# ilur98/DLMC-QUANT

Hardware: AMD Instinct MI355X
Metric: ResNet-50 W8A8 fake-quant fwd images/sec (higher is better)
Workload: dtype i8; 1 GPU; resnet50 W8A8 per-channel fake-quant forward (FSPTQ forms: W minmax_channel s8, A minmax_tensor u8), BN folded first as in FSPTQuant.py:67, fused int8 MFMA conv/linear, frozen execution plan (epilogue-fused ReLU / shortcut / next-layer codes; block end + next 1x1 as one launch; weight codes quantised once at plan build), 2 HIP streams per GPU, 224x224 relu(N(0,1)) pixels, batch 512 per GPU, scales; global_batch=512, parallelism=dp1 (batch-sharded replicas)

## Files before the change

dlmc-quant_amd/csrc/conv_pw_i8.hip:

```cpp
#include "conv_i8_common.h"

namespace dlmcq {

struct PwArgs {
  const int8_t* x;
  const int8_t* w;
  const float* s_w;
  const int32_t* wsum;
  const float* bias;
  const float* s_in;
  const float* zp_in;
  int M, K, shift, nslice;
  int nblk;
  unsigned long long* trace;
};

constexpr int PW_WPS(int c, int bn) { return c >= 1024 ? 1 : (c >= 512 ? 3 : 4); }

template <int C, int BN, int NTP, bool ASYM, int NW, int LAB = 0, bool R6 = false>
__global__ __launch_bounds__(NW * 64, PW_WPS(C, BN)) void conv_pw_i8_kernel(PwArgs a, ConvEpi ep) {
  constexpr int S = C / 64;
  constexpr int NA = C / 32;
  constexpr int NT = BN / 32;
  constexpr int WB = C * BN;
  constexpr int PIECES = S * (BN / 16);
  constexpr int NPAR = ASYM ? 4 : 3;
  constexpr int NP = NT / NTP;
  constexpr int JP = NTP > 1 ? 1 : 0;
  static_assert(NT % NTP == 0 && JP < NTP && NTP >= 1, "the request sits inside the last pass's epilogue");
  extern __shared__ __attribute__((aligned(1024))) int8_t pw_lds[];
  int8_t* const wl = pw_lds;
  int8_t* const par = pw_lds + WB;
  constexpr int SROW = BN + 16;
  constexpr int LPR = BN / 16, RPI = 64 / LPR;
  constexpr int NST = (32 + RPI - 1) / RPI;
  int8_t* const stg = pw_lds + WB + 4 * BN * 4 + (threadIdx.x >> 6) * (32 * SROW);
  const int srow = (int)((threadIdx.x & 63) / LPR), sseg = (int)(threadIdx.x & 63) - srow * LPR;

  const int tid = threadIdx.x, wave = tid >> 6, lane = tid & 63, l31 = lane & 31, hsel = lane >> 5;
  const uint32_t b = blockIdx.x;
  const int slice = (int)((b >> 3) % (uint32_t)a.nslice);
  const int group = (int)((b >> 3) / (uint32_t)a.nslice) * 8 + (int)(b & 7u);
  const int ngroups = (int)(gridDim.x / (uint32_t)a.nslice);
  const int n0 = slice * BN;

  unsigned long long* tr = nullptr;
  if (LAB == 1 && a.trace && blockIdx.x == gridDim.x / 2 && tid == 0) tr = a.trace;
  int nstamp = 3;
  auto stamp = [&]() {
    if (LAB == 1 && tr && nstamp < 256) tr[nstamp++] = __builtin_readcyclecounter();
  };
  if (LAB == 1 && tr) tr[0] = __builtin_amdgcn_s_memrealtime();
  stamp();
  unsigned long long* wgt = nullptr;
  if (LAB == 1 && a.trace && tid == 0) {
    wgt = a.trace + 256 + 4 * (size_t)blockIdx.x;
    wgt[0] = __builtin_amdgcn_s_memrealtime();
    wgt[2] = __builtin_amdgcn_s_getreg(4 | (31 << 11));
    wgt[3] = __builtin_amdgcn_s_getreg(20 | (31 << 11));
  }
  {
    const void* arrs[4] = {a.s_w, a.wsum, a.bias, ASYM ? ep.w_off : nullptr};
#pragma unroll
    for (int r = 0; r < NPAR; ++r) {
      if (!arrs[r]) {
        for (int c = tid; c < BN; c += NW * 64) reinterpret_cast<float*>(par)[r * BN + c] = 0.0f;
        continue;
      }
      for (int c = wave; c < BN / 64; c += NW)
        __builtin_amdgcn_global_load_lds((gptr_t)(static_cast<const int32_t*>(arrs[r]) + n0 + c * 64 + lane), (lptr_t)(par + (r * BN + c * 64) * 4), 4, 0, 0);
    }
    const int lrow = lane >> 2, pslot = lane & 3;
    for (int pc = wave; pc < PIECES; pc += NW) {
      const int s = pc / (BN / 16), r16 = pc - s * (BN / 16);
      const int row = r16 * 16 + lrow;
      const int d = row & 31;
      const int k = n0 + (row & ~31) + 16 * ((d >> 2) & 1) + 4 * (d >> 3) + (d & 3);
      const int seg = pslot ^ ((row >> 2) & 3);
      __builtin_amdgcn_global_load_lds((gptr_t)(a.w + (int64_t)k * C + s * 64 + seg * 16), (lptr_t)(wl + s * (BN * 64) + r16 * 1024), 16, 0, 0);
    }
  }
  const float zpf = a.zp_in ? a.zp_in[0] : 0.0f;
  const int zpi = (int)__builtin_rintf(zpf);
  const float sin = a.s_in[0];
  const uint32_t xorw = a.shift ? 0x80808080u : 0u;
  const EpiQuant eq(ep, ep.relu != 0);
  const v4i r_x = make_rsrc(a.x, (uint32_t)((int64_t)a.M * C));
  const v4i r_c = make_rsrc(ep.codes, (uint32_t)((int64_t)a.M * a.K));

  i32x4 areg[NA];
  auto request = [&](int blk) {
    const int row = blk * 32 + l31;
    const int vo = (blk < a.nblk && row < a.M) ? row * C + hsel * 16 : BUF_BIG;
    if constexpr (LAB == 2) {
#pragma unroll
      for (int f = 0; f < NA; ++f) areg[f] = i32x4{vo, 1, 2, 3};
      return;
    }
    static_for<NA>([&](auto f) { bload16i<decltype(f)::value * 32>(areg[decltype(f)::value], vo, r_x); });
  };
  const int stride = ngroups * NW;
  int blk = group * NW + wave;
  request(blk);
  asm volatile("s_waitcnt vmcnt(0)" ::: "memory");
  __syncthreads();
  if (tid < BN) {
    float* pf = reinterpret_cast<float*>(par) + tid;
    int* pi = reinterpret_cast<int*>(par) + BN + tid;
    *pf = sin * *pf;
    *pi = (a.shift - zpi) * *pi;
    if constexpr (ASYM) pf[3 * BN] = sin * pf[3 * BN];
  }
  __syncthreads();

  stamp();
  for (; blk < a.nblk; blk += stride) {
    stamp();
    if constexpr (LAB == 2 || LAB == 7 || LAB == 8) asm volatile("s_waitcnt vmcnt(0)" ::: "memory");
    else asm volatile("s_waitcnt vmcnt(%0)" ::"n"(NST) : "memory");
    stamp();
#pragma unroll
    for (int f = 0; f < NA; ++f) {
      asm volatile("" : "+v"(areg[f]));
      areg[f] = i32x4{(int)(areg[f].x ^ xorw), (int)(areg[f].y ^ xorw), (int)(areg[f].z ^ xorw), (int)(areg[f].w ^ xorw)};
    }
    f32x2 s0f2 = f32x2{0.0f, 0.0f};
    static_for<NP>([&](auto p_c) {
      constexpr int p = decltype(p_c)::value;
      i32x16 acc[NTP];
#pragma unroll
      for (int j = 0; j < NTP; ++j) {
        const i32x4* cop = reinterpret_cast<const i32x4*>(par + (BN + (p * NTP + j) * 32 + hsel * 16) * 4);
#pragma unroll
        for (int q = 0; q < 4; ++q) {
          const i32x4 c4 = cop[q];
          acc[j][4 * q] = c4.x;
          acc[j][4 * q + 1] = c4.y;
          acc[j][4 * q + 2] = c4.z;
          acc[j][4 * q + 3] = c4.w;
        }
      }
      int s0 = 0;
      static_for<NA>([&](auto f_c) {
        constexpr int f = decltype(f_c)::value;
        constexpr int s = f >> 1, ks = f & 1;
        const i32x4 af = areg[f];
        if constexpr (ASYM && p == 0) {
          s0 = __builtin_amdgcn_sdot4(af.x, 0x01010101, s0, false);
          s0 = __builtin_amdgcn_sdot4(af.y, 0x01010101, s0, false);
          s0 = __builtin_amdgcn_sdot4(af.z, 0x01010101, s0, false);
          s0 = __builtin_amdgcn_sdot4(af.w, 0x01010101, s0, false);
        }
        const int sg = ks * 2 + hsel;
#pragma unroll
        for (int j = 0; j < NTP; ++j) {
          const int brow = (p * NTP + j) * 32 + l31;
          const i32x4 bf = *reinterpret_cast<const i32x4*>(wl + s * (BN * 64) + brow * 64 + ((sg ^ ((brow >> 2) & 3)) << 4));
          if constexpr (LAB == 4) asm volatile("" ::"v"(af), "v"(bf));
          else acc[j] = __builtin_amdgcn_mfma_i32_32x32x32_i8(bf, af, acc[j], 0, 0, 0);
        }
      });
      if constexpr (LAB == 1) {
        asm volatile("s_nop 0" ::"v"(acc[0][0]), "v"(acc[NTP - 1][15]));
        stamp();
      }
      if constexpr (ASYM && p == 0) {
        s0 += __shfl_xor(s0, 32, 64);
        s0 += (a.shift - zpi) * C;
        s0f2 = f32x2{(float)s0, (float)s0};
      }
#pragma unroll
      for (int jj = 0; jj < NTP; ++jj) {
        if (p == NP - 1 && jj == JP) request(blk + stride);
        const int j = p * NTP + jj;
        const int cb = j * 32 + hsel * 16;
        if constexpr (LAB == 6 || LAB == 7) {
          uint32_t wl4[4];
#pragma unroll
          for (int q = 0; q < 4; ++q)
            wl4[q] = (uint32_t)(acc[jj][4 * q] & 0xff) | ((uint32_t)(acc[jj][4 * q + 1] & 0xff) << 8) | ((uint32_t)(acc[jj][4 * q + 2] & 0xff) << 16) |
                     ((uint32_t)acc[jj][4 * q + 3] << 24);
          if constexpr (LAB == 6) *reinterpret_cast<i32x4*>(stg + l31 * SROW + cb) = i32x4{(int)wl4[0], (int)wl4[1], (int)wl4[2], (int)wl4[3]};
          else asm volatile("" ::"v"(wl4[0]), "v"(wl4[1]), "v"(wl4[2]), "v"(wl4[3]));
          continue;
        }
        f32x4 y[4];
#pragma unroll
        for (int q = 0; q < 4; ++q) {
          const f32x4 mu = *reinterpret_cast<const f32x4*>(par + (cb + 4 * q) * 4);
          const f32x4 bs = *reinterpret_cast<const f32x4*>(par + (2 * BN + cb + 4 * q) * 4);
          f32x2 ya = pk_fma(f32x2{(float)acc[jj][4 * q], (float)acc[jj][4 * q + 1]}, f32x2{mu.x, mu.y}, f32x2{bs.x, bs.y});
          f32x2 yb = pk_fma(f32x2{(float)acc[jj][4 * q + 2], (float)acc[jj][4 * q + 3]}, f32x2{mu.z, mu.w}, f32x2{bs.z, bs.w});
          if constexpr (ASYM) {
            const f32x4 wo = *reinterpret_cast<const f32x4*>(par + (3 * BN + cb + 4 * q) * 4);
            ya = ya + s0f2 * f32x2{wo.x, wo.y};
            yb = yb + s0f2 * f32x2{wo.z, wo.w};
          }
          y[q] = f32x4{ya.x, ya.y, yb.x, yb.y};
          if constexpr (R6) y[q] = cap6_nan4(y[q]);
        }
        uint32_t wq[4];
        eq.code4n_plain(y, wq);
        *reinterpret_cast<i32x4*>(stg + l31 * SROW + cb) = i32x4{(int)wq[0], (int)wq[1], (int)wq[2], (int)wq[3]};
      }
      stamp();
    });
    if constexpr (LAB != 7) {
      const int r0 = blk * 32 + srow;
      const int vbase = r0 * a.K + n0 + sseg * 16;
      const int8_t* const sbase = stg + srow * SROW + sseg * 16;
#pragma unroll
      for (int it = 0; it < NST; ++it) {
        const bool ok = srow < RPI && it * RPI + srow < 32 && r0 + it * RPI < a.M;
        const bool whole = (it + 1) * RPI <= 32;
        const i32x4 c16 = *reinterpret_cast<const i32x4*>(whole || it * RPI + srow < 32 ? sbase + it * RPI * SROW : stg + 31 * SROW + sseg * 16);
        if constexpr (LAB == 8) asm volatile("" ::"v"(c16));
        else if constexpr (LAB == 9) bstore16i_nt(c16, ok ? vbase + it * RPI * a.K : BUF_BIG, r_c);
        else bstore16i(c16, ok ? vbase + it * RPI * a.K : BUF_BIG, r_c);
      }
    }
    stamp();
  }
  if (LAB == 1 && tr) {
    asm volatile("s_waitcnt vmcnt(0)" ::: "memory");
    stamp();
    tr[1] = __builtin_amdgcn_s_memrealtime();
    tr[2] = (unsigned long long)nstamp;
  }
  if (LAB == 1 && wgt) {
    asm volatile("s_waitcnt vmcnt(0)" ::: "memory");
    wgt[1] = __builtin_amdgcn_s_memrealtime();
  }
  asm volatile("s_waitcnt vmcnt(0)" ::: "memory");
}

#define DLMCQ_PW_PAIRS(X) X(64, 64) X(64, 128) X(64, 192) X(128, 128) X(128, 192) X(192, 128) X(192, 192) X(512, 128) X(1024, 128)
constexpr int pw_slice(int64_t K) { return K == 192 ? 192 : (K == 64 ? 64 : (K % 128 == 0 ? 128 : 0)); }
constexpr bool pw_built(int64_t C, int bn) {
#define DLMCQ_PW_HAS(CC, BB) if (C == CC && bn == BB) return true;
  DLMCQ_PW_PAIRS(DLMCQ_PW_HAS)
#undef DLMCQ_PW_HAS
  return false;
}

bool conv_pw_applies(int64_t N, int64_t H, int64_t W, int64_t C, int64_t K, int64_t R, int64_t S, int32_t stride, int32_t pad,
                     int32_t dilation, const ConvEpi& ep, const float* out, bool dual) {
  if (R != 1 || S != 1 || stride != 1 || pad != 0 || dilation != 1 || dual || out || ep.residual || !ep.codes) return false;
  if (!epi_plain(ep)) return false;
  if (K > 1024 || !pw_built(C, pw_slice(K))) return false;
  if (!aligned16(ep.codes)) return false;
  const int64_t M = N * H * W;
  if (M < 4096) return false;
  if (M * C >= (int64_t)BUF_BIG || M * K >= (int64_t)BUF_BIG) return false;
  return true;
}

template <int C, int BN, bool ASYM, int LAB = 0, bool R6 = false>
static int pw_go(const PwArgs& a0, const ConvEpi& ep, hipStream_t st) {
  constexpr int WPS = PW_WPS(C, BN);
  constexpr int LDS1 = C * BN + 4 * BN * 4, STG = 4 * 32 * (BN + 16);
  constexpr bool BIGWG = C >= 1024 || (LDS1 + STG) * WPS > 158 * 1024;
  constexpr int NW = C >= 1024 ? 6 : (BIGWG ? 4 * WPS : 4);
  constexpr int LDS = LDS1 + NW * (STG / 4);
  static_assert(LDS <= 160 * 1024, "LDS");
  PwArgs a = a0;
  a.nslice = a.K / BN;
  static int cus = 0;
  if (!cus) {
    int dev = 0;
    hipDeviceProp_t prop;
    cus = (hipGetDevice(&dev) == hipSuccess && hipGetDeviceProperties(&prop, dev) == hipSuccess && prop.multiProcessorCount > 0)
              ? prop.multiProcessorCount : 256;
  }
  const int wgs = cus * (BIGWG ? 1 : WPS);
  int ngroups = (wgs / a.nslice) & ~7;
  if (ngroups < 8) ngroups = 8;
  const int maxg = ((a.nblk + NW - 1) / NW + 7) & ~7;
  if (ngroups > maxg) ngroups = maxg;
  constexpr int NTP = BN == 192 ? 3 : (C >= 512 ? 1 : 2);
  auto kern = conv_pw_i8_kernel<C, BN, NTP, ASYM, NW, LAB, R6>;
  static bool attr_set = false;
  if (!attr_set) {
    const hipError_t e = hipFuncSetAttribute(reinterpret_cast<const void*>(kern), hipFuncAttributeMaxDynamicSharedMemorySize, LDS);
    if (e != hipSuccess) return (int)e;
    attr_set = true;
  }
  hipLaunchKernelGGL(kern, dim3((uint32_t)(ngroups * a.nslice)), dim3(NW * 64), LDS, st, a, ep);
  return launch_status();
}

int conv_pw_launch(const int8_t* x, const int8_t* w, const float* bias, const int32_t* wsum, const float* in_scale,
                   const float* in_zero_point, const float* w_scale, int64_t N, int64_t H, int64_t W, int64_t C, int64_t K, int shift,
                   const ConvEpi& ep, hipStream_t st, int lab, void* lab_trace) {
  PwArgs a{};
  a.trace = static_cast<unsigned long long*>(lab_trace);
  a.x = x; a.w = w; a.s_w = w_scale; a.wsum = wsum; a.bias = bias; a.s_in = in_scale; a.zp_in = in_zero_point;
  a.M = (int)(N * H * W); a.K = (int)K; a.shift = shift;
  a.nblk = (a.M + 31) / 32;
  const bool asym = ep.w_off != nullptr;
  const int bn = pw_slice(K);
#ifdef DLMCQ_LAB
#define DLMCQ_PWL(CC, BB, L) \
  if (C == CC && bn == BB && lab == L && asym) return pw_go<CC, BB, true, L>(a, ep, st)
#define DLMCQ_PWLS(CC, BB) DLMCQ_PWL(CC, BB, 1); DLMCQ_PWL(CC, BB, 2); DLMCQ_PWL(CC, BB, 4); DLMCQ_PWL(CC, BB, 6); DLMCQ_PWL(CC, BB, 7); DLMCQ_PWL(CC, BB, 8); DLMCQ_PWL(CC, BB, 9)
  DLMCQ_PWLS(128, 128);
  DLMCQ_PWLS(192, 192);
  DLMCQ_PWLS(192, 128);
  DLMCQ_PWLS(512, 128);
#undef DLMCQ_PWLS
#undef DLMCQ_PWL
#endif
  if (lab) return DLMCQ_EINVAL;
  const bool r6 = ep.relu == DLMCQ_ACT_RELU6;
#define DLMCQ_PW(CC, BB)                                                                                       \
  if (C == CC && bn == BB)                                                                                     \
    return r6 ? (asym ? pw_go<CC, BB, true, 0, true>(a, ep, st) : pw_go<CC, BB, false, 0, true>(a, ep, st))     \
              : (asym ? pw_go<CC, BB, true>(a, ep, st) : pw_go<CC, BB, false>(a, ep, st));
  DLMCQ_PW_PAIRS(DLMCQ_PW)
#undef DLMCQ_PW
  return DLMCQ_EINVAL;
}

}
```

Measured before the change: 94170 images/s.

## Split pointwise conv K-loop into double-buffered halves for wide-C layers

Adds a KH template parameter that splits the activation fragments of the pointwise int8 kernel into KH parts, alternating between two register sets. The next part's loads are issued before the current part's MFMAs, so global loads overlap compute. This targets C=1024 and C=2048 inputs in ResNet-50, which now use a 64-wide output slice and a 2- or 4-way split, and C=2048 is newly routed to this kernel. The cost is more register pressure and different occupancy (two waves per SIMD). The epilogue is moved into a lambda and the CU count is now read through a shared helper.

```diff
diff --git a/dlmc-quant_amd/csrc/conv_pw_i8.hip b/dlmc-quant_amd/csrc/conv_pw_i8.hip
--- a/dlmc-quant_amd/csrc/conv_pw_i8.hip
+++ b/dlmc-quant_amd/csrc/conv_pw_i8.hip
@@ -15,12 +15,13 @@
   unsigned long long* trace;
 };
 
-constexpr int PW_WPS(int c, int bn) { return c >= 1024 ? 1 : (c >= 512 ? 3 : 4); }
-
-template <int C, int BN, int NTP, bool ASYM, int NW, int LAB = 0, bool R6 = false>
-__global__ __launch_bounds__(NW * 64, PW_WPS(C, BN)) void conv_pw_i8_kernel(PwArgs a, ConvEpi ep) {
+constexpr int PW_WPS(int c, int bn, int kh = 1) { return kh > 1 ? 2 : (c >= 1024 ? 1 : (c >= 512 ? 3 : 4)); }
+
+template <int C, int BN, int NTP, bool ASYM, int NW, int LAB = 0, bool R6 = false, int KH = 1>
+__global__ __launch_bounds__(NW * 64, PW_WPS(C, BN, KH)) void conv_pw_i8_kernel(PwArgs a, ConvEpi ep) {
   constexpr int S = C / 64;
   constexpr int NA = C / 32;
+  constexpr int NAH = NA / KH;
   constexpr int NT = BN / 32;
   constexpr int WB = C * BN;
   constexpr int PIECES = S * (BN / 16);
@@ -28,6 +29,7 @@
   constexpr int NP = NT / NTP;
   constexpr int JP = NTP > 1 ? 1 : 0;
   static_assert(NT % NTP == 0 && JP < NTP && NTP >= 1, "the request sits inside the last pass's epilogue");
+  static_assert(KH == 1 || (KH % 2 == 0 && NA % KH == 0 && NTP == NT && LAB == 0), "parts alternate between two fragment sets; one pass");
   extern __shared__ __attribute__((aligned(1024))) int8_t pw_lds[];
   int8_t* const wl = pw_lds;
   int8_t* const par = pw_lds + WB;
@@ -88,20 +90,22 @@
   const v4i r_x = make_rsrc(a.x, (uint32_t)((int64_t)a.M * C));
   const v4i r_c = make_rsrc(ep.codes, (uint32_t)((int64_t)a.M * a.K));
 
-  i32x4 areg[NA];
-  auto request = [&](int blk) {
+  i32x4 areg[KH > 1 ? 2 : 1][NAH];
+  auto request = [&](int blk, auto h_c, auto set_c) {
+    constexpr int h = decltype(h_c)::value, set = decltype(set_c)::value;
     const int row = blk * 32 + l31;
     const int vo = (blk < a.nblk && row < a.M) ? row * C + hsel * 16 : BUF_BIG;
     if constexpr (LAB == 2) {
 #pragma unroll
-      for (int f = 0; f < NA; ++f) areg[f] = i32x4{vo, 1, 2, 3};
+      for (int f = 0; f < NAH; ++f) areg[set][f] = i32x4{vo, 1, 2, 3};
       return;
     }
-    static_for<NA>([&](auto f) { bload16i<decltype(f)::value * 32>(areg[decltype(f)::value], vo, r_x); });
+    static_for<NAH>([&](auto f) { bload16i<(h * NAH + decltype(f)::value) * 32>(areg[set][decltype(f)::value], vo, r_x); });
   };
+  constexpr std::integral_constant<int, 0> i0{};
   const int stride = ngroups * NW;
   int blk = group * NW + wave;
-  request(blk);
+  request(blk, i0, i0);
   asm volatile("s_waitcnt vmcnt(0)" ::: "memory");
   __syncthreads();
   if (tid < BN) {
@@ -113,17 +117,53 @@
   }
   __syncthreads();
 
+  auto finish = [&](const i32x16& accj, const int j, const f32x2 s0f2) {
+    const int cb = j * 32 + hsel * 16;
+    if constexpr (LAB == 6 || LAB == 7) {
+      uint32_t wl4[4];
+#pragma unroll
+      for (int q = 0; q < 4; ++q)
+        wl4[q] = (uint32_t)(accj[4 * q] & 0xff) | ((uint32_t)(accj[4 * q + 1] & 0xff) << 8) | ((uint32_t)(accj[4 * q + 2] & 0xff) << 16) |
+                 ((uint32_t)accj[4 * q + 3] << 24);
+      if constexpr (LAB == 6) *reinterpret_cast<i32x4*>(stg + l31 * SROW + cb) = i32x4{(int)wl4[0], (int)wl4[1], (int)wl4[2], (int)wl4[3]};
+      else asm volatile("" ::"v"(wl4[0]), "v"(wl4[1]), "v"(wl4[2]), "v"(wl4[3]));
+      return;
+    }
+    f32x4 y[4];
+#pragma unroll
+    for (int q = 0; q < 4; ++q) {
+      const f32x4 mu = *reinterpret_cast<const f32x4*>(par + (cb + 4 * q) * 4);
+      const f32x4 bs = *reinterpret_cast<const f32x4*>(par + (2 * BN + cb + 4 * q) * 4);
+      f32x2 ya = pk_fma(f32x2{(float)accj[4 * q], (float)accj[4 * q + 1]}, f32x2{mu.x, mu.y}, f32x2{bs.x, bs.y});
+      f32x2 yb = pk_fma(f32x2{(float)accj[4 * q + 2], (float)accj[4 * q + 3]}, f32x2{mu.z, mu.w}, f32x2{bs.z, bs.w});
+      if constexpr (ASYM) {
+        const f32x4 wo = *reinterpret_cast<const f32x4*>(par + (3 * BN + cb + 4 * q) * 4);
+        ya = ya + s0f2 * f32x2{wo.x, wo.y};
+        yb = yb + s0f2 * f32x2{wo.z, wo.w};
+      }
+      y[q] = f32x4{ya.x, ya.y, yb.x, yb.y};
+      if constexpr (R6) y[q] = cap6_nan4(y[q]);
+    }
+    uint32_t wq[4];
+    eq.code4n_plain(y, wq);
+    *reinterpret_cast<i32x4*>(stg + l31 * SROW + cb) = i32x4{(int)wq[0], (int)wq[1], (int)wq[2], (int)wq[3]};
+  };
+  auto landed = [&](auto set_c, auto cnt_c) {
+    constexpr int set = decltype(set_c)::value;
+    if constexpr (LAB == 2 || LAB == 7 || LAB == 8) asm volatile("s_waitcnt vmcnt(0)" ::: "memory");
+    else asm volatile("s_waitcnt vmcnt(%0)" ::"n"(decltype(cnt_c)::value) : "memory");
+    stamp();
+#pragma unroll
+    for (int f = 0; f < NAH; ++f) {
+      asm volatile("" : "+v"(areg[set][f]));
+      areg[set][f] = i32x4{(int)(areg[set][f].x ^ xorw), (int)(areg[set][f].y ^ xorw), (int)(areg[set][f].z ^ xorw),
+                           (int)(areg[set][f].w ^ xorw)};
+    }
+  };
   stamp();
   for (; blk < a.nblk; blk += stride) {
     stamp();
-    if constexpr (LAB == 2 || LAB == 7 || LAB == 8) asm volatile("s_waitcnt vmcnt(0)" ::: "memory");
-    else asm volatile("s_waitcnt vmcnt(%0)" ::"n"(NST) : "memory");
-    stamp();
-#pragma unroll
-    for (int f = 0; f < NA; ++f) {
-      asm volatile("" : "+v"(areg[f]));
-      areg[f] = i32x4{(int)(areg[f].x ^ xorw), (int)(areg[f].y ^ xorw), (int)(areg[f].z ^ xorw), (int)(areg[f].w ^ xorw)};
-    }
+    if constexpr (KH == 1) landed(i0, std::integral_constant<int, NST>{});
     f32x2 s0f2 = f32x2{0.0f, 0.0f};
     static_for<NP>([&](auto p_c) {
       constexpr int p = decltype(p_c)::value;
@@ -141,24 +181,32 @@
         }
       }
       int s0 = 0;
-      static_for<NA>([&](auto f_c) {
-        constexpr int f = decltype(f_c)::value;
-        constexpr int s = f >> 1, ks = f & 1;
-        const i32x4 af = areg[f];
-        if constexpr (ASYM && p == 0) {
-          s0 = __builtin_amdgcn_sdot4(af.x, 0x01010101, s0, false);
-          s0 = __builtin_amdgcn_sdot4(af.y, 0x01010101, s0, false);
-          s0 = __builtin_amdgcn_sdot4(af.z, 0x01010101, s0, false);
-          s0 = __builtin_amdgcn_sdot4(af.w, 0x01010101, s0, false);
+      static_for<KH>([&](auto h_c) {
+        constexpr int h = decltype(h_c)::value, set = h & 1;
+        if constexpr (KH > 1) {
+          if constexpr (h + 1 < KH) request(blk, std::integral_constant<int, h + 1>{}, std::integral_constant<int, (h + 1) & 1>{});
+          else request(blk + stride, i0, i0);
+          landed(std::integral_constant<int, set>{}, std::integral_constant<int, (h == 0 ? NST : 0) + NAH>{});
         }
-        const int sg = ks * 2 + hsel;
-#pragma unroll
-        for (int j = 0; j < NTP; ++j) {
-          const int brow = (p * NTP + j) * 32 + l31;
-          const i32x4 bf = *reinterpret_cast<const i32x4*>(wl + s * (BN * 64) + brow * 64 + ((sg ^ ((brow >> 2) & 3)) << 4));
-          if constexpr (LAB == 4) asm volatile("" ::"v"(af), "v"(bf));
-          else acc[j] = __builtin_amdgcn_mfma_i32_32x32x32_i8(bf, af, acc[j], 0, 0, 0);
-        }
+        static_for<NAH>([&](auto f_c) {
+          constexpr int f = h * NAH + decltype(f_c)::value;
+          constexpr int s = f >> 1, ks = f & 1;
+          const i32x4 af = areg[set][decltype(f_c)::value];
+          if constexpr (ASYM && p == 0) {
+            s0 = __builtin_amdgcn_sdot4(af.x, 0x01010101, s0, false);
+            s0 = __builtin_amdgcn_sdot4(af.y, 0x01010101, s0, false);
+            s0 = __builtin_amdgcn_sdot4(af.z, 0x01010101, s0, false);
+            s0 = __builtin_amdgcn_sdot4(af.w, 0x01010101, s0, false);
+          }
+          const int sg = ks * 2 + hsel;
+#pragma unroll
+          for (int j = 0; j < NTP; ++j) {
+            const int brow = (p * NTP + j) * 32 + l31;
+            const i32x4 bf = *reinterpret_cast<const i32x4*>(wl + s * (BN * 64) + brow * 64 + ((sg ^ ((brow >> 2) & 3)) << 4));
+            if constexpr (LAB == 4) asm volatile("" ::"v"(af), "v"(bf));
+            else acc[j] = __builtin_amdgcn_mfma_i32_32x32x32_i8(bf, af, acc[j], 0, 0, 0);
+          }
+        });
       });
       if constexpr (LAB == 1) {
         asm volatile("s_nop 0" ::"v"(acc[0][0]), "v"(acc[NTP - 1][15]));
@@ -171,37 +219,8 @@
       }
 #pragma unroll
       for (int jj = 0; jj < NTP; ++jj) {
-        if (p == NP - 1 && jj == JP) request(blk + stride);
-        const int j = p * NTP + jj;
-        const int cb = j * 32 + hsel * 16;
-        if constexpr (LAB == 6 || LAB == 7) {
-          uint32_t wl4[4];
-#pragma unroll
-          for (int q = 0; q < 4; ++q)
-            wl4[q] = (uint32_t)(acc[jj][4 * q] & 0xff) | ((uint32_t)(acc[jj][4 * q + 1] & 0xff) << 8) | ((uint32_t)(acc[jj][4 * q + 2] & 0xff) << 16) |
-                     ((uint32_t)acc[jj][4 * q + 3] << 24);
-          if constexpr (LAB == 6) *reinterpret_cast<i32x4*>(stg + l31 * SROW + cb) = i32x4{(int)wl4[0], (int)wl4[1], (int)wl4[2], (int)wl4[3]};
-          else asm volatile("" ::"v"(wl4[0]), "v"(wl4[1]), "v"(wl4[2]), "v"(wl4[3]));
-          continue;
-        }
-        f32x4 y[4];
-#pragma unroll
-        for (int q = 0; q < 4; ++q) {
-          const f32x4 mu = *reinterpret_cast<const f32x4*>(par + (cb + 4 * q) * 4);
-          const f32x4 bs = *reinterpret_cast<const f32x4*>(par + (2 * BN + cb + 4 * q) * 4);
-          f32x2 ya = pk_fma(f32x2{(float)acc[jj][4 * q], (float)acc[jj][4 * q + 1]}, f32x2{mu.x, mu.y}, f32x2{bs.x, bs.y});
-          f32x2 yb = pk_fma(f32x2{(float)acc[jj][4 * q + 2], (float)acc[jj][4 * q + 3]}, f32x2{mu.z, mu.w}, f32x2{bs.z, bs.w});
-          if constexpr (ASYM) {
-            const f32x4 wo = *reinterpret_cast<const f32x4*>(par + (3 * BN + cb + 4 * q) * 4);
-            ya = ya + s0f2 * f32x2{wo.x, wo.y};
-            yb = yb + s0f2 * f32x2{wo.z, wo.w};
-          }
-          y[q] = f32x4{ya.x, ya.y, yb.x, yb.y};
-          if constexpr (R6) y[q] = cap6_nan4(y[q]);
-        }
-        uint32_t wq[4];
-        eq.code4n_plain(y, wq);
-        *reinterpret_cast<i32x4*>(stg + l31 * SROW + cb) = i32x4{(int)wq[0], (int)wq[1], (int)wq[2], (int)wq[3]};
+        if (KH == 1 && p == NP - 1 && jj == JP) request(blk + stride, i0, i0);
+        finish(acc[jj], p * NTP + jj, s0f2);
       }
       stamp();
     });
@@ -234,10 +253,16 @@
   asm volatile("s_waitcnt vmcnt(0)" ::: "memory");
 }
 
-#define DLMCQ_PW_PAIRS(X) X(64, 64) X(64, 128) X(64, 192) X(128, 128) X(128, 192) X(192, 128) X(192, 192) X(512, 128) X(1024, 128)
-constexpr int pw_slice(int64_t K) { return K == 192 ? 192 : (K == 64 ? 64 : (K % 128 == 0 ? 128 : 0)); }
-constexpr bool pw_built(int64_t C, int bn) {
-#define DLMCQ_PW_HAS(CC, BB) if (C == CC && bn == BB) return true;
+#define DLMCQ_PW_PAIRS(X)                                                                                                            \
+  X(64, 64, 1, true) X(64, 128, 1, true) X(64, 192, 1, true) X(128, 128, 1, true) X(128, 192, 1, true) X(192, 128, 1, true)          \
+  X(192, 192, 1, true) X(512, 128, 1, true) X(1024, 128, 1, true) X(1024, 64, 2, true) X(2048, 64, 4, false)
+constexpr int pw_slice(int64_t C, int64_t K) {
+  if ((C == 1024 || C == 2048) && K % 128 == 0 && K <= 512) return 64;
+  if (C == 2048) return 0;
+  return K == 192 ? 192 : (K == 64 ? (C < 1024 ? 64 : 0) : (K % 128 == 0 ? 128 : 0));
+}
+constexpr bool pw_built(int64_t C, int bn, bool asym) {
+#define DLMCQ_PW_HAS(CC, BB, HH, AS) if (C == CC && bn == BB) return AS || !asym;
   DLMCQ_PW_PAIRS(DLMCQ_PW_HAS)
 #undef DLMCQ_PW_HAS
   return false;
@@ -247,7 +272,7 @@
                      int32_t dilation, const ConvEpi& ep, const float* out, bool dual) {
   if (R != 1 || S != 1 || stride != 1 || pad != 0 || dilation != 1 || dual || out || ep.residual || !ep.codes) return false;
   if (!epi_plain(ep)) return false;
-  if (K > 1024 || !pw_built(C, pw_slice(K))) return false;
+  if (K > 1024 || !pw_built(C, pw_slice(C, K), ep.w_off != nullptr)) return false;
   if (!aligned16(ep.codes)) return false;
   const int64_t M = N * H * W;
   if (M < 4096) return false;
@@ -255,30 +280,23 @@
   return true;
 }
 
-template <int C, int BN, bool ASYM, int LAB = 0, bool R6 = false>
+template <int C, int BN, bool ASYM, int LAB = 0, bool R6 = false, int KH = 1>
 static int pw_go(const PwArgs& a0, const ConvEpi& ep, hipStream_t st) {
-  constexpr int WPS = PW_WPS(C, BN);
+  constexpr int WPS = PW_WPS(C, BN, KH);
   constexpr int LDS1 = C * BN + 4 * BN * 4, STG = 4 * 32 * (BN + 16);
   constexpr bool BIGWG = C >= 1024 || (LDS1 + STG) * WPS > 158 * 1024;
-  constexpr int NW = C >= 1024 ? 6 : (BIGWG ? 4 * WPS : 4);
+  constexpr int NW = KH > 1 ? 4 * WPS : (C >= 1024 ? 6 : (BIGWG ? 4 * WPS : 4));
   constexpr int LDS = LDS1 + NW * (STG / 4);
   static_assert(LDS <= 160 * 1024, "LDS");
   PwArgs a = a0;
   a.nslice = a.K / BN;
-  static int cus = 0;
-  if (!cus) {
-    int dev = 0;
-    hipDeviceProp_t prop;
-    cus = (hipGetDevice(&dev) == hipSuccess && hipGetDeviceProperties(&prop, dev) == hipSuccess && prop.multiProcessorCount > 0)
-              ? prop.multiProcessorCount : 256;
-  }
-  const int wgs = cus * (BIGWG ? 1 : WPS);
+  const int wgs = device_cus() * (BIGWG ? 1 : WPS);
   int ngroups = (wgs / a.nslice) & ~7;
   if (ngroups < 8) ngroups = 8;
   const int maxg = ((a.nblk + NW - 1) / NW + 7) & ~7;
   if (ngroups > maxg) ngroups = maxg;
-  constexpr int NTP = BN == 192 ? 3 : (C >= 512 ? 1 : 2);
-  auto kern = conv_pw_i8_kernel<C, BN, NTP, ASYM, NW, LAB, R6>;
+  constexpr int NTP = KH > 1 ? BN / 32 : (BN == 192 ? 3 : (C >= 512 ? 1 : 2));
+  auto kern = conv_pw_i8_kernel<C, BN, NTP, ASYM, NW, LAB, R6, KH>;
   static bool attr_set = false;
   if (!attr_set) {
     const hipError_t e = hipFuncSetAttribute(reinterpret_cast<const void*>(kern), hipFuncAttributeMaxDynamicSharedMemorySize, LDS);
@@ -287,6 +305,16 @@
   }
   hipLaunchKernelGGL(kern, dim3((uint32_t)(ngroups * a.nslice)), dim3(NW * 64), LDS, st, a, ep);
   return launch_status();
+}
+
+template <int C, int BN, int KH, bool AS>
+static int pw_pick(const PwArgs& a, const ConvEpi& ep, hipStream_t st) {
+  const bool r6 = ep.relu == DLMCQ_ACT_RELU6;
+  if (ep.w_off != nullptr) {
+    if constexpr (AS) return r6 ? pw_go<C, BN, true, 0, true, KH>(a, ep, st) : pw_go<C, BN, true, 0, false, KH>(a, ep, st);
+    else return DLMCQ_EINVAL;
+  }
+  return r6 ? pw_go<C, BN, false, 0, true, KH>(a, ep, st) : pw_go<C, BN, false, 0, false, KH>(a, ep, st);
 }
 
 int conv_pw_launch(const int8_t* x, const int8_t* w, const float* bias, const int32_t* wsum, const float* in_scale,
@@ -297,9 +325,9 @@
   a.x = x; a.w = w; a.s_w = w_scale; a.wsum = wsum; a.bias = bias; a.s_in = in_scale; a.zp_in = in_zero_point;
   a.M = (int)(N * H * W); a.K = (int)K; a.shift = shift;
   a.nblk = (a.M + 31) / 32;
+  const int bn = pw_slice(C, K);
+#ifdef DLMCQ_LAB
   const bool asym = ep.w_off != nullptr;
-  const int bn = pw_slice(K);
-#ifdef DLMCQ_LAB
 #define DLMCQ_PWL(CC, BB, L) \
   if (C == CC && bn == BB && lab == L && asym) return pw_go<CC, BB, true, L>(a, ep, st)
 #define DLMCQ_PWLS(CC, BB) DLMCQ_PWL(CC, BB, 1); DLMCQ_PWL(CC, BB, 2); DLMCQ_PWL(CC, BB, 4); DLMCQ_PWL(CC, BB, 6); DLMCQ_PWL(CC, BB, 7); DLMCQ_PWL(CC, BB, 8); DLMCQ_PWL(CC, BB, 9)
@@ -311,11 +339,8 @@
 #undef DLMCQ_PWL
 #endif
   if (lab) return DLMCQ_EINVAL;
-  const bool r6 = ep.relu == DLMCQ_ACT_RELU6;
-#define DLMCQ_PW(CC, BB)                                                                                       \
-  if (C == CC && bn == BB)                                                                                     \
-    return r6 ? (asym ? pw_go<CC, BB, true, 0, true>(a, ep, st) : pw_go<CC, BB, false, 0, true>(a, ep, st))     \
-              : (asym ? pw_go<CC, BB, true>(a, ep, st) : pw_go<CC, BB, false>(a, ep, st));
+#define DLMCQ_PW(CC, BB, HH, AS) \
+  if (C == CC && bn == BB) return pw_pick<CC, BB, HH, AS>(a, ep, st);
   DLMCQ_PW_PAIRS(DLMCQ_PW)
 #undef DLMCQ_PW
   return DLMCQ_EINVAL;
```

Result: slower. 93010 images/s (-1.2%).
